# saforem2/l2hmc

Hardware: AMD Instinct MI355X
Metric: leapfrog-steps/sec (whole node), 8x8 U(1) batch 2048, 10 LF (higher is better)
Workload: dtype f32; 1 GPU; U(1) 8x8 lattice, beta=2.0, batch 2048 per GPU, 10 LF steps, GenericNet H=512 (BASELINE.json configs[2]); global_batch=2048, num_steps=10, parallelism=chains sharded over 1 GPU(s) (weak scaling), weights replicated

## Files before the change

include/l2hmc_hip.h:

```cpp
#ifndef L2HMC_HIP_H
#define L2HMC_HIP_H

#include <stddef.h>
#include <stdint.h>

#ifdef __cplusplus
extern "C" {
#endif

#define L2HMC_OK 0
#define L2HMC_ERR_ARG 1
#define L2HMC_ERR_HIP 2
#define L2HMC_ERR_WORKSPACE 3

#define L2HMC_ABI_VERSION 1

typedef void* l2hmc_stream_t;

int l2hmc_abi_version(void);
const char* l2hmc_last_error(void);

int l2hmc_u1_action_force(const float* x, int64_t rows, int32_t T, int32_t X, float beta,
                          float* action, float* force, float* avg_plaq, float* top_charge,
                          l2hmc_stream_t stream);
// ... 38 lines not shown

int l2hmc_stq_dense(const l2hmc_dense_net* net, const float* a, const float* b, const float* bmask,
                    float t_cos, float t_sin, int64_t rows, float* S, float* T, float* Q,
                    void* ws, size_t ws_bytes, l2hmc_stream_t stream);

size_t l2hmc_stq_conv3d_ws_bytes(int64_t rows, int32_t H, int32_t T, int32_t X, int32_t F);
int l2hmc_stq_conv3d(const l2hmc_conv3d_front* front, const l2hmc_dense_net* net, int32_t T, int32_t X,
                     const float* a, const float* b, const float* bmask, float t_cos, float t_sin,
                     int64_t rows, float* S, float* Tr, float* Q, void* ws, size_t ws_bytes,
                     l2hmc_stream_t stream);

int l2hmc_lf_update_v(const float* v, const float* grad, const float* S, const float* T,
                      const float* Q, float eps, int32_t dir, int64_t rows, int32_t D,
                      float* v_out, float* logdet, l2hmc_stream_t stream);
int l2hmc_lf_update_x(const float* x, const float* v, const float* keep, const float* S,
                      const float* T, const float* Q, float eps, int32_t dir, int64_t rows,
                      int32_t D, float* x_out, float* logdet, l2hmc_stream_t stream);

int l2hmc_accept_prob(const float* h_old, const float* h_new, const float* sumlogdet, int64_t n,
                      float* p, l2hmc_stream_t stream);

int l2hmc_mix_accept(const float* x, const float* xf, const float* vf, const float* pf,
                     const float* xb, const float* vb, const float* pb, const float* coin,
                     const float* u, int32_t strict, int64_t B, int32_t D, float* x_prop,
                     float* v_prop, float* p, float* x_out, l2hmc_stream_t stream);

#define L2HMC_PLAN_LAYERED 1
#define L2HMC_PLAN_CONV3D 2
#define L2HMC_PLAN_SELECTED_ONLY 4
#define L2HMC_PLAN_RECOMPUTE 8
#define L2HMC_PLAN_TILES16_ONLY 16
#define L2HMC_PLAN_ALL_COLUMNS 32
#define L2HMC_PLAN_FULL_L1 64
typedef struct l2hmc_gauge_plan {
  int32_t T, X;
  int32_t num_steps;
  int32_t hmc;
  float eps;
  int32_t flags;
  const float* masks;
  l2hmc_dense_net xnet;
  l2hmc_dense_net vnet;
  l2hmc_conv3d_front xfront;
  l2hmc_conv3d_front vfront;
  const void* heads;
} l2hmc_gauge_plan;

size_t l2hmc_gauge_pack_heads_bytes(const l2hmc_gauge_plan* plan);
int l2hmc_gauge_pack_heads(const l2hmc_gauge_plan* plan, void* heads, l2hmc_stream_t stream);

size_t l2hmc_gauge_ws_bytes(const l2hmc_gauge_plan* plan, int64_t rows);

int l2hmc_gauge_plan_fused(const l2hmc_gauge_plan* plan);

int l2hmc_gauge_step_plan(int64_t rows_all, int32_t cus, int64_t* rows_out, int32_t* rows_per_wg_out);

int l2hmc_gauge_leapfrog(const l2hmc_gauge_plan* plan, float beta, int32_t step, float* x, float* v,
                         const int32_t* dir, int64_t rows, float* logdet, void* ws, size_t ws_bytes,
                         l2hmc_stream_t stream);

int l2hmc_gauge_trajectory(const l2hmc_gauge_plan* plan, float beta, const float* x0, const float* v0,
                           const int32_t* dir, int64_t rows, float* x_out, float* v_out,
                           float* sumlogdet, float* p_accept, void* ws, size_t ws_bytes,
                           l2hmc_stream_t stream);

size_t l2hmc_gauge_transition_ws_bytes(const l2hmc_gauge_plan* plan, int64_t B, int32_t both_directions);
// ... 178 lines not shown
```

l2hmc_amd/_lib.py:

```python
import ctypes as C
import os
import re

import torch

_HERE = os.path.dirname(os.path.abspath(__file__))
LIB_PATH = os.environ.get("L2HMC_LIB_PATH") or os.path.join(_HERE, "libl2hmc_hip.so")
HEADER_PATH = os.path.join(os.path.dirname(_HERE), "include", "l2hmc_hip.h")

c_float_p = C.c_void_p
MAX_MIX, MAX_SMALL_DIM, MAX_SMALL_NODES = 8, 8, 64
PLAN_LAYERED, PLAN_CONV3D, PLAN_SELECTED_ONLY, PLAN_RECOMPUTE, PLAN_TILES16_ONLY, PLAN_ALL_COLUMNS = 1, 2, 4, 8, 16, 32
PLAN_FULL_L1 = 64
GRAD_BUCKET_REST = 6
BUCKET_FN = C.CFUNCTYPE(None, C.c_void_p, C.c_int32)


class DenseNet(C.Structure):
    _fields_ = [("D", C.c_int32), ("H", C.c_int32), ("Ka", C.c_int32), ("Kb", C.c_int32),
                ("w1_t", c_float_p), ("wt", c_float_p), ("b1", c_float_p), ("wh_t", c_float_p),
                ("bh", c_float_p), ("whd_t", c_float_p), ("bhd", c_float_p),
                ("coeff_s", c_float_p), ("coeff_q", c_float_p),
                ("q_tanh", C.c_int32), ("reserved", C.c_int32), ("packed", c_float_p)]


class DenseGrads(C.Structure):
    _fields_ = [(n, c_float_p) for n in ("w1_t", "wt", "b1", "wh_t", "bh", "whd_t", "bhd", "coeff_s", "coeff_q")]


class Conv3DGrads(C.Structure):
    _fields_ = [(n, c_float_p) for n in ("w1_a", "b1_a", "w2_a", "b2_a", "w1_b", "b1_b", "w2_b", "b2_b")]


class Conv3DFront(C.Structure):
    _fields_ = [("F", C.c_int32), ("reserved", C.c_int32),
                ("w1_a", c_float_p), ("b1_a", c_float_p), ("w2_a", c_float_p), ("b2_a", c_float_p),
                ("w1_b", c_float_p), ("b1_b", c_float_p), ("w2_b", c_float_p), ("b2_b", c_float_p)]


class GaugePlan(C.Structure):
    _fields_ = [("T", C.c_int32), ("X", C.c_int32), ("num_steps", C.c_int32), ("hmc", C.c_int32),
                ("eps", C.c_float), ("flags", C.c_int32), ("masks", c_float_p),
                ("xnet", DenseNet), ("vnet", DenseNet), ("xfront", Conv3DFront), ("vfront", Conv3DFront),
                ("heads", C.c_void_p)]


# ... 211 lines not shown
```

l2hmc_amd/csrc/fused_args.h:

```cpp
#pragma once
#include "stq_dense.h"

namespace l2hmc {

struct FusedArgs {
  int T, X, num_steps, step_begin, step_end;
  float eps, beta;
  const float* masks;
  l2hmc_dense_net xnet, vnet;
  l2hmc_conv3d_front xfront, vfront;
  const float* x0; const float* v0;
  const int* dir;
  int64_t x_mod;
  int64_t dir_split;
  int64_t rows;
  float* x_out; float* v_out;
  float* logdet;
  int logdet_accumulate;
  float* p_accept;
  unsigned long long* stamps;
  int stagger;
  FusedTape tx, tv;
  float* step_x_next;
  float* step_xprop; float* step_vprop; float* step_xout;
  int64_t step_B;
  int64_t step_Bl, step_chain0;
  int step_sums_acc;
  unsigned long long step_seed, step_draw;
  int step_both;
  float* step_px; float* step_act; float* step_plq; float* step_chg; float* step_dq;
  float* step_sums;
  float* step_part;
  int step_split;
  float* step_hand;
  int* step_ticket;
  const int* heads_meta;
  const float* heads_img;
  const float* l1_img;
};

size_t fused4_pack_floats(const l2hmc_dense_net* n);
int launch_fused4_pack(const l2hmc_dense_net* n, float* image4, hipStream_t stream);
int fused4_rows_per_wg(int64_t rows, int cus);
int launch_fused4(const FusedArgs& a, int rows_per_wg, hipStream_t stream);

int fused32_supported(const l2hmc_dense_net* n);
int launch_fused32(const FusedArgs& a, hipStream_t stream);

}
```

l2hmc_amd/csrc/fused_traj.hip:

```cpp
#include "fused_step.h"
#include "lf_update.h"
#include <atomic>
#include <stdlib.h>

namespace l2hmc {

template <int D, int H, int KA = D, bool CONV = false>
struct FusedCfg {
  static constexpr int IMGW = CONV ? 2 * kFWaves : kFWaves;
  static constexpr int WAVES = 2 * kFWaves;
  static constexpr int RW = WAVES / IMGW;
  static constexpr int THREADS = 64 * WAVES;
  static constexpr int TPC = CONV ? THREADS / kFM : 16;
  static constexpr int SX = D + 8;
  static constexpr int SA = KA + 8;
  static constexpr int SH = H + 8;
  static constexpr int NT1 = H / (16 * WAVES);
  static constexpr int NTH = D / (16 * WAVES);
  static constexpr int NTI1 = H / (16 * IMGW);
  static constexpr int NTIH = D / (16 * IMGW);
  static_assert(NT1 >= 1 && NT1 <= 8 && NTH >= 1, "every wave needs at least one tile per layer");
  static_assert(RW == 1 || NTH == 1, "a shared heads section is walked with one tile per head and wave");
  static constexpr int KC1 = 2 * KA / 16;
  static constexpr int KC2 = H / 16;
  static constexpr size_t P1 = (size_t)2 * KA * H;
  static constexpr size_t P2 = (size_t)H * H;
  static constexpr size_t PH = (size_t)3 * D * H;
  static constexpr int NC = 4 * H + 5 * D;
  static constexpr int CF = 8, CL = 8;
  static constexpr int CW = 18 * CF + CF + 8 * CF * CF + 2 * CF;
  static constexpr int CXIN = (CL + 2) * (CL + 2) * 2;
  static constexpr int CP1 = (CL / 2 + 1) * (CL / 2 + 1) * CF;
  static constexpr int CONV_FLOATS = CONV ? 2 * kFM * SA + 4 * CW + kFM * (CXIN + CP1) : 0;
  static constexpr int ACT_FLOATS = CONV ? 0 : kFM * SX + D + 4 + D + 2 * kFM;
  static constexpr int LDS_FLOATS = 3 * kFM * SX + 2 * kFM * SH + 2 * NC + kFM * (D / 2 + 4)  +
                                    2 * D  + WAVES * kFM  + (RW > 1 ? IMGW * 64 : 0)  + kFM  +
                                    8 * kFM  + CONV_FLOATS + ACT_FLOATS;
};

__global__ void pack_fused_kernel(l2hmc_dense_net n, float* __restrict__ out, int waves) {
  const int kFWaves = waves;
  const int D = n.D, H = n.H, K1 = n.Ka + n.Kb;
  const size_t P1 = (size_t)K1 * H, P2 = (size_t)H * H, PH = (size_t)3 * D * H;
  const int NT1 = H / (16 * kFWaves), NTH = D / (16 * kFWaves);
  for (size_t i = (size_t)blockIdx.x * blockDim.x + threadIdx.x; i < P1 + P2 + PH;
       i += (size_t)gridDim.x * blockDim.x) {
    const int j = (int)(i & 3), lane = (int)((i >> 2) & 63);
    size_t rest;
    float val;
    if (i < P1 + P2) {
      const bool first = i < P1;
      const int K = first ? K1 : H;
      rest = (first ? i : i - P1) >> 8;
      const int t = (int)(rest % NT1);
      rest /= NT1;
      const int KC = K / 16;
      const int kc = (int)(rest % KC), w = (int)(rest / KC);
      const int col = (w * NT1 + t) * 16 + (lane & 15);
      const int k = kc * 16 + (lane >> 4) * 4 + j;
      val = first ? n.w1_t[(size_t)col * K1 + k] : n.wh_t[(size_t)col * H + k];
    } else {
      rest = (i - P1 - P2) >> 8;
      const int t = (int)(rest % NTH);
      rest /= NTH;
      const int hd = (int)(rest % 3);
      rest /= 3;
      const int KC = H / 16;
// ... 86 lines not shown
    __builtin_amdgcn_sched_barrier(0);                                                        \
    t_;                                                                                       \
  })
#define FT_ADD(slot, t0) ft[slot] += FT_NOW() - (t0)
#else
#define FT_NOW() 0ull
#define FT_ADD(slot, t0) do {} while (0)
#endif


#ifdef L2HMC_STAMPS
int g_fused_stagger = 0;
extern "C" void l2hmc_debug_set_stagger(int cycles) { g_fused_stagger = cycles; }
#endif

template <int D, int H, int KA, bool CONV, bool TAPE = false>
__global__ __launch_bounds__((FusedCfg<D, H, KA, CONV>::THREADS)) void gauge_traj_fused_kernel(FusedArgs p) {
  using Cfg = FusedCfg<D, H, KA, CONV>;
  constexpr int kFWaves = Cfg::WAVES, kFThreads = Cfg::THREADS, kTPC = Cfg::TPC;
  constexpr int SX = Cfg::SX, SH = Cfg::SH, SA = Cfg::SA, NT1 = Cfg::NT1, NTH = Cfg::NTH;
  constexpr int RW = Cfg::RW, IMGW = Cfg::IMGW, NTI1 = Cfg::NTI1, NTIH = Cfg::NTIH;
  constexpr int TSH = RW > 1 ? NTIH : 1;
  constexpr int sites = D / 2;
  constexpr int SP = sites + 4;
  extern __shared__ __attribute__((aligned(16))) float lds[];
  float* xs = lds;
  float* vs = xs + kFM * SX;
  float* gs = vs + kFM * SX;
  float* h1 = gs + kFM * SX;
  float* h2 = h1 + kFM * SH;
  float* cx = h2 + kFM * SH;
  float* cv = cx + Cfg::NC;
  float* sp = cv + Cfg::NC;
  float* skm = sp + kFM * SP;
  float* ldw = skm + 2 * D;
  float* ldx = ldw + IMGW * kFM;
  int* sdir = reinterpret_cast<int*>(ldw + kFWaves * kFM + (RW > 1 ? IMGW * 64 : 0));
  float* stp = reinterpret_cast<float*>(sdir + kFM);
  float* fa = stp + 8 * kFM;
  float* fb = fa + kFM * SA;
  float* cwl = fb + kFM * SA;
  float* cxin = cwl + 4 * Cfg::CW;
  float* cp1 = cxin + kFM * Cfg::CXIN;
  float* stg = stp + 8 * kFM + Cfg::CONV_FLOATS;
  int* scol = reinterpret_cast<int*>(stg + kFM * SX);
  int* sel = scol + D;
  int* scp = sel + 4;
  float* spz = reinterpret_cast<float*>(scp + D);

  [[maybe_unused]] unsigned long long ft[10] = {0, 0, 0, 0, 0, 0, 0, 0, 0, 0};
  [[maybe_unused]] const unsigned long long ft_start = FT_NOW();
#ifdef L2HMC_STAMPS
  unsigned long long rt0;
  asm volatile("s_memrealtime %0\n\ts_waitcnt lgkmcnt(0)" : "=s"(rt0)::"memory");
#endif
  const int tid = threadIdx.x;
  const int lane = tid & 63, wave = tid >> 6;
  const int q = lane >> 4, r = lane & 15;
  const int64_t row0 = (int64_t)blockIdx.x * kFM;
  const int nrow = (int)min((int64_t)kFM, p.rows - row0);
  const float eps = p.eps;

#ifdef L2HMC_STAMPS
  if (p.stagger > 0) {
    const long long delay = (long long)((blockIdx.x >> 3) & 31) * p.stagger;
    const long long t0 = (long long)__builtin_amdgcn_s_memtime();
    while ((long long)__builtin_amdgcn_s_memtime() - t0 < delay) __builtin_amdgcn_s_sleep(16);
  }
#endif
  const bool SPLIT = !CONV && !TAPE && p.step_B > 0 && p.step_both && p.step_split;
  const StepWg wg = step_workgroup<kFM>(p, stp, SPLIT);
  const bool STEPM = wg.stepm;
  const int sdw = wg.sdw;
  float* spx = wg.spx;
  stage_chains<kFM, kFThreads, D, SX>(p, wg, xs, vs, sdir);
  load_consts<kFThreads, D, H>(p.xnet, cx, tid);
  load_consts<kFThreads, D, H>(p.vnet, cv, tid);
  if constexpr (CONV) {
    constexpr int F = Cfg::CF, F2 = 2 * Cfg::CF;
    auto load_filters = [&](const float* w1, const float* b1, const float* w2, const float* b2, float* dst) {
      for (int i = tid; i < 18 * F; i += kFThreads) dst[i] = w1[i];
// ... 101 lines not shown
          for (int wi = 0; wi < 3; ++wi)
#pragma unroll
            for (int wj = 0; wj < 3; ++wj)
              w[wi][wj] = *reinterpret_cast<const f32x4*>(pbase + (wi * L2P + wj) * F + ch4);
#pragma unroll
          for (int di = 0; di < 2; ++di)
#pragma unroll
            for (int dj = 0; dj < 2; ++dj)
#pragma unroll
              for (int cc = 0; cc < 4; ++cc) {
                const f32x2 kw = *reinterpret_cast<const f32x2*>(w2 + ((di * 2 + dj) * F + ch4 + cc) * F2 + 2 * gp);
#pragma unroll
                for (int a = 0; a < 2; ++a)
#pragma unroll
                  for (int bb = 0; bb < 2; ++bb) {
                    const float xv = w[a + di][bb + dj][cc];
                    acc[a][bb] += f32x2{xv, xv} * kw;
                  }
              }
        }
        const float m0 = fmaxf(fmaxf(acc[0][0][0], acc[0][1][0]), fmaxf(acc[1][0][0], acc[1][1][0]));
        const float m1 = fmaxf(fmaxf(acc[0][0][1], acc[0][1][1]), fmaxf(acc[1][0][1], acc[1][1][1]));
        *reinterpret_cast<f32x2*>(dst + c * SA + (I2 * L4 + J2) * F2 + 2 * gp) = f32x2{fmaxf(m0, 0.f), fmaxf(m1, 0.f)};
      }
    }
    __syncthreads();
  };

  f32x4 keep_v[NT1], keep_x[NT1];
  bool keep_v_valid = false;
  constexpr bool ACTOK = !CONV && !TAPE && Cfg::NTH == 1 && RW == 2 && kFWaves == 8;
  int arow = 0;

  auto net_update = [&](const l2hmc_dense_net& net, const float* cn, const float* in1, int mode, int sub,
                        bool prep_next_mask, int l1, bool is_vnet, const float tcr, const float tsr,
                        int callidx) {
    const float* pk = net.packed;
    const bool zig = (callidx & 1) != 0;
    [[maybe_unused]] const FusedTape& tp = is_vnet ? p.tv : p.tx;
    [[maybe_unused]] const size_t tcr0 = (size_t)callidx * (size_t)p.rows + (size_t)row0;
    if constexpr (TAPE) {
      {
        const float* stsrc = mode == 1 ? vs : xs;
        for (int i = tid; i < kFM * (D / 4); i += kFThreads) {
          const int rr = i / (D / 4), c4 = (i - rr * (D / 4)) * 4;
          if (rr < nrow) {
            float* dst = tp.in + (tcr0 + rr) * (2 * D);
            tape_store(dst + c4, *reinterpret_cast<const f32x4*>(in1 + rr * SX + c4));
            tape_store(dst + D + c4, *reinterpret_cast<const f32x4*>(gs + rr * SX + c4));
            tape_store(tp.st + (tcr0 + rr) * D + c4, *reinterpret_cast<const f32x4*>(stsrc + rr * SX + c4));
          }
        }
      }
    }
    [[maybe_unused]] auto tape_rows = [&](float* dst, const float* src) {
      for (int i = tid; i < kFM * (H / 4); i += kFThreads) {
        const int rr = i / (H / 4), c4 = (i - rr * (H / 4)) * 4;
        if (rr < nrow)
          tape_store(dst + (tcr0 + rr) * H + c4, *reinterpret_cast<const f32x4*>(src + rr * SH + c4));
      }
    };
    const int wv = __builtin_amdgcn_readfirstlane(wave);
    const int wimg = wv / RW, wsub = wv - wimg * RW;
    const float* wp1 = pk + (size_t)wimg * Cfg::KC1 * NTI1 * 256;
    const float* wp2 = pk + Cfg::P1 + (size_t)wimg * Cfg::KC2 * NTI1 * 256;
    const float* wph = pk + Cfg::P1 + Cfg::P2 + (size_t)wimg * Cfg::KC2 * 3 * NTIH * 256;
    const int to1 = wsub * NT1, toh = wsub * NTH;
    int asense = 0;
    bool actv = false;
    const float* wpa = nullptr;
    if (ACTOK && SPLIT && mode == 2 && p.heads_img) {
      asense = sdw ^ sub;
      actv = __builtin_amdgcn_readfirstlane(sel[asense]) != 0;
      wpa = p.heads_img + ((size_t)(arow * 2 + asense) * 4 + (wv & 3)) * Cfg::KC2 * 3 * 256;
    }
    const bool l1c = ACTOK && SPLIT && p.l1_img && p.heads_img && __builtin_amdgcn_readfirstlane(sel[0] & sel[1]) != 0;
    [[maybe_unused]] float ld_k[4] = {0.f, 0.f, 0.f, 0.f}, ld_s[4] = {0.f, 0.f, 0.f, 0.f};
#ifndef L2HMC_DP1
#define L2HMC_DP1 3
#define L2HMC_DP2 3
#define L2HMC_DPH 4
#endif
    constexpr int DP1 = L2HMC_DP1, DP2 = L2HMC_DP2, DPH = L2HMC_DPH;
    BRing<NT1, DP2> R2;
    BRing<3 * NTH, DPH> R3;
    {
      constexpr int KH = Cfg::KC1 / 2;
      f32x4 acc[NT1];
      [[maybe_unused]] unsigned long long t0 = FT_NOW();
      const float* src1 = in1;
      const float* src2 = gs;
      int s1 = SX;
      if constexpr (CONV) {
        const float* cwn = cwl + (is_vnet ? 2 : 0) * Cfg::CW;
        [[maybe_unused]] const unsigned long long tc0 = FT_NOW();
        if (l1 == 0 || l1 == 1 || l1 == 3) conv_features(in1, cwn, fa);
        if (l1 != 2) conv_features(gs, cwn + Cfg::CW, fb);
        FT_ADD(8, tc0);
        src1 = fa;
        src2 = fb;
        s1 = SA;
        if constexpr (TAPE) {
          for (int i = tid; i < kFM * (2 * KA / 4); i += kFThreads) {
            const int rr = i / (2 * KA / 4), c4 = (i - rr * (2 * KA / 4)) * 4;
            if (rr < nrow)
              tape_store(tp.feat + (tcr0 + rr) * (2 * KA) + c4,
                         *reinterpret_cast<const f32x4*>((c4 < KA ? fa + rr * SA + c4 : fb + rr * SA + (c4 - KA))));
          }
        }
      }
      if (l1 == 2) {
#pragma unroll
        for (int t = 0; t < NT1; ++t) acc[t] = keep_v[t];
      } else {
        BRing<NT1, DP1> RA, RB;
        const bool cmp = l1c && mode == 2;
        const float* wpb = wp1 + (size_t)KH * NTI1 * 256;
        if (cmp) wpb = p.l1_img + ((size_t)(arow * 2 + asense) * IMGW + wimg) * (KH / 2) * NTI1 * 256;
        ring_prime<NT1, DP1, NTI1>(RB, wpb, false, 0, to1);
        if (l1 == 4) {
#pragma unroll
          for (int t = 0; t < NT1; ++t) acc[t] = keep_x[t];
// ... 8 lines not shown
#pragma unroll
            for (int t = 0; t < NT1; ++t) keep_x[t] = acc[t];
          }
        }
        bool x_done = false;
        if constexpr (ACTOK) {
          if (cmp) {
            x_done = true;
            const float* a2 = (sub == 0 ? stg : gs) + r * SX + q * 4;
            const bool bad = spz[sub * kFM + r] != 0.f;
            stream_layer<NT1, KH / 2, DP1, NTI1>(
                RB, wpb,
                [&](int kc) {
                  f32x4 a = *reinterpret_cast<const f32x4*>(a2 + kc * 16);
                  if (kc == 0) {
#pragma unroll
                    for (int e = 0; e < 4; ++e) a[e] = bad ? __builtin_nanf("") : a[e];
                  }
                  return a;
                },
                acc, false, to1);
          }
        }
        if (!x_done) {
          const float* a2 = src2 + r * s1 + q * 4;
          stream_layer<NT1, KH, DP1, NTI1>(
              RB, wpb, [&](int kc) { return *reinterpret_cast<const f32x4*>(a2 + kc * 16); }, acc, false, to1);
        }
        if (l1 == 1) {
#pragma unroll
          for (int t = 0; t < NT1; ++t) keep_v[t] = acc[t];
        }
      }
      ring_prime<NT1, DP2, NTI1>(R2, wp2, zig, Cfg::KC2, to1);
      FT_ADD(0, t0);
      t0 = FT_NOW();
      [[maybe_unused]] unsigned gmask = 0;
#pragma unroll
      for (int t = 0; t < NT1; ++t) {
        const int c0 = (wave * NT1 + t) * 16 + q * 4;
        const f32x4 b = *reinterpret_cast<const f32x4*>(cn + c0);
        const f32x4 w0 = *reinterpret_cast<const f32x4*>(cn + H + c0);
        const f32x4 w1 = *reinterpret_cast<const f32x4*>(cn + 2 * H + c0);
        f32x4 hv;
#pragma unroll
        for (int e = 0; e < 4; ++e) {
          hv[e] = fmaxf(acc[t][e] + b[e] + (tcr * w0[e] + tsr * w1[e]), 0.f);
          if constexpr (TAPE) gmask |= (hv[e] > 0.f ? 1u : 0u) << (t * 4 + e);
        }
        *reinterpret_cast<f32x4*>(h1 + r * SH + c0) = hv;
      }
      if constexpr (TAPE) {
        const size_t word = ((size_t)(callidx * 2 + 0) * gridDim.x + blockIdx.x) * (64 * IMGW) + wimg * 64 + lane;
        if constexpr (RW == 1) tp.gate[word] = gmask;
        else reinterpret_cast<unsigned short*>(tp.gate)[word * 2 + wsub] = (unsigned short)gmask;
      }
      FT_ADD(3, t0);
    }
    {
      [[maybe_unused]] const unsigned long long tb = FT_NOW();
      __syncthreads();
      FT_ADD(6, tb);
    }
    if constexpr (TAPE) tape_rows(tp.h1, h1);
    {
      f32x4 acc[NT1];
#pragma unroll
      for (int t = 0; t < NT1; ++t) acc[t] = f32x4{0.f, 0.f, 0.f, 0.f};
      const float* a = h1 + r * SH + q * 4;
      [[maybe_unused]] unsigned long long t0 = FT_NOW();
      stream_layer<NT1, Cfg::KC2, DP2, NTI1>(
          R2, wp2, [&](int kc) { return *reinterpret_cast<const f32x4*>(a + kc * 16); }, acc, zig, to1);
      if (ACTOK && actv) {
        if (wv < 4) ring_prime<3 * NTH, DPH, 3, 1>(R3, wpa, zig, Cfg::KC2, 0);
      } else {
        ring_prime<3 * NTH, DPH, 3 * NTIH, TSH>(R3, wph, zig, Cfg::KC2, toh);
      }
      FT_ADD(1, t0);
      t0 = FT_NOW();
      [[maybe_unused]] unsigned gmask = 0;
#pragma unroll
      for (int t = 0; t < NT1; ++t) {
        const int c0 = (wave * NT1 + t) * 16 + q * 4;
        const f32x4 b = *reinterpret_cast<const f32x4*>(cn + 3 * H + c0);
        f32x4 hv;
#pragma unroll
        for (int e = 0; e < 4; ++e) {
          hv[e] = fmaxf(acc[t][e] + b[e], 0.f);
          if constexpr (TAPE) gmask |= (hv[e] > 0.f ? 1u : 0u) << (t * 4 + e);
        }
        *reinterpret_cast<f32x4*>(h2 + r * SH + c0) = hv;
      }
      if constexpr (TAPE) {
        const size_t word = ((size_t)(callidx * 2 + 1) * gridDim.x + blockIdx.x) * (64 * IMGW) + wimg * 64 + lane;
        if constexpr (RW == 1) tp.gate[word] = gmask;
        else reinterpret_cast<unsigned short*>(tp.gate)[word * 2 + wsub] = (unsigned short)gmask;
      }
      FT_ADD(4, t0);
    }
    {
      [[maybe_unused]] const unsigned long long tb = FT_NOW();
      __syncthreads();
      FT_ADD(6, tb);
    }
    if constexpr (TAPE) tape_rows(tp.h2, h2);
    {
      f32x4 acc[3 * NTH];
#pragma unroll
      for (int t = 0; t < 3 * NTH; ++t) acc[t] = f32x4{0.f, 0.f, 0.f, 0.f};
      const float* a = h2 + r * SH + q * 4;
      [[maybe_unused]] unsigned long long t0 = FT_NOW();
      if (ACTOK && actv) {
        if (wv < 4)
          stream_layer<3 * NTH, Cfg::KC2, DPH, 3, 1>(
              R3, wpa, [&](int kc) { return *reinterpret_cast<const f32x4*>(a + kc * 16); }, acc, zig, 0);
      } else {
        stream_layer<3 * NTH, Cfg::KC2, DPH, 3 * NTIH, TSH>(
            R3, wph, [&](int kc) { return *reinterpret_cast<const f32x4*>(a + kc * 16); }, acc, zig, toh);
      }
      FT_ADD(2, t0);
      t0 = FT_NOW();
      float ld = 0.f;
      const float* bhd = cn + 4 * H;
      const float* es = bhd + 3 * D;
      const float* eq = es + D;
      const int d = dirl;
      if (ACTOK && actv) {
        const int* al = scol + asense * (D / 2);
        const int* il = scol + (asense ^ 1) * (D / 2);
        if (wv < 4) {
#pragma unroll
          for (int e = 0; e < 4; ++e) {
            const int c = al[wv * 16 + q * 4 + e];
            const int idx = r * SX + c;
            float S, Tt, Q, s, omk;
            heads_stq(acc[0][e], acc[1][e], acc[2][e], bhd[c], bhd[D + c], bhd[2 * D + c], es[c], eq[c], net.q_tanh, S,
                      Tt, Q);
            const float xn = lf_drift<ExpFast>(xs[idx], vs[idx], keep_of(skm[c], skm[D + c], d, sub), S, Tt, Q, eps, d, s,
                                               omk);
            xs[idx] = xn;
            stg[idx] = omk * s;
            if (prep_next_mask) gs[l1c ? r * SX + scp[c] : idx] = omk * xn;
          }
        } else {
#pragma unroll
          for (int e = 0; e < 4; ++e) {
            const int c = il[(wv - 4) * 16 + q * 4 + e];
            const int idx = r * SX + c;
            stg[idx] = 0.f;
            if (prep_next_mask) {
              const float kx = (1.f - keep_of(skm[c], skm[D + c], d, sub)) * xs[idx];
              if (!l1c) gs[idx] = kx;
              else if (kx != kx) spz[kFM + r] = kx;
// ... 82 lines not shown
      }
      }
      FT_ADD(5, t0);
    }
    {
      [[maybe_unused]] const unsigned long long tb = FT_NOW();
      __syncthreads();
      FT_ADD(6, tb);
    }
    if (ACTOK && actv) {
      if (wsub == 1) {
        float ld = 0.f;
#pragma unroll
        for (int h = 0; h < 2; ++h)
#pragma unroll
          for (int e = 0; e < 4; ++e) ld += stg[r * SX + (2 * wimg + h) * 16 + q * 4 + e];
        ld += __shfl_xor(ld, 16, 64);
        ld += __shfl_xor(ld, 32, 64);
        if (q == 0) ldw[wimg * kFM + r] += ld;
      }
    } else if constexpr (RW > 1) {
      if (wsub == 1) {
        float ld = ldx[wimg * 64 + lane];
#pragma unroll
        for (int e = 0; e < 4; ++e) ld += ld_k[e] * ld_s[e];
        ld += __shfl_xor(ld, 16, 64);
        ld += __shfl_xor(ld, 32, 64);
        if (q == 0) ldw[wimg * kFM + r] += ld;
      }
    }
  };

  const float two_pi = 6.28318530717958647692f;
  for (int step = p.step_begin; step < p.step_end; ++step) {
    const int sf = step, sb = p.num_steps - 1 - step;
    const float af = two_pi * (float)sf / (float)p.num_steps, ab = two_pi * (float)sb / (float)p.num_steps;
    const float tcf = cosf(af), tsf = sinf(af), tcb = cosf(ab), tsb = sinf(ab);
    const float tcr = dirl ? tcb : tcf, tsr = dirl ? tsb : tsf;
    for (int i = tid; i < D; i += kFThreads) {
      skm[i] = p.masks[(size_t)sf * D + i];
      skm[D + i] = p.masks[(size_t)sb * D + i];
    }
    if (ACTOK && SPLIT && p.heads_meta) {
      arow = sdw ? sb : sf;
      for (int i = tid; i < D; i += kFThreads) scol[i] = p.heads_meta[2 * p.num_steps + arow * D + i];
      if (tid < 2) sel[tid] = p.heads_meta[arow * 2 + tid];
      if (p.l1_img)
        for (int i = tid; i < D; i += kFThreads) scp[i] = p.heads_meta[2 * p.num_steps + (p.num_steps + arow) * D + i];
    }
    __syncthreads();
#pragma nounroll
    for (int call = 0; call < 4; ++call) {
      const bool is_v = call == 0 || call == 3;
      if (call == 3) {
        [[maybe_unused]] const unsigned long long tf = FT_NOW();
        float unused[1];
        force_pass<kFM, kTPC, 1, D, SX, SP>(cl, xs, sp, gs, unused);
        FT_ADD(7, tf);
      }
      const int l1 = call == 0 ? (keep_v_valid ? 2 : 0) : call == 1 ? 3 : call == 2 ? 4 : 1;
      net_update(is_v ? p.vnet : p.xnet, is_v ? cv : cx, is_v ? xs : vs, is_v ? 1 : 2, call == 2 ? 1 : 0,
                 call < 2, l1, is_v, tcr, tsr, 2 * step + (call == 0 || call == 1 ? 0 : 1));
    }
    keep_v_valid = true;
  }

  float act1[1], kin1[1];
  force_pass<kFM, kTPC, 1, D, SX, SP>(cl, xs, sp, gs, act1);
  kinetic_pass<kFM, kTPC, 1, D, SX>(cl, vs, kin1);
  if (STEPM) {
    step_accept_probs<kFM, 1, IMGW>(cl, ldw, act0, act1, kin0, kin1, spx);
    __syncthreads();
    const float* xfr = xs;
    const float* xbr = xs + (kFM / 2) * SX;
    const float* vfr = vs;
    const float* vbr = vs + (kFM / 2) * SX;
    const float* pfr = spx;
    const float* pbr = spx + kFM / 2;
    if (SPLIT) {
      constexpr int HW = 2 * kFM * D + kFM;
      float* mine = p.step_hand + (size_t)blockIdx.x * HW;
      for (int i = tid; i < kFM * (D / 4); i += kFThreads) {
        const int rr = i / (D / 4), c4 = (i - rr * (D / 4)) * 4;
        *reinterpret_cast<f32x4*>(mine + rr * D + c4) = *reinterpret_cast<const f32x4*>(xs + rr * SX + c4);
        if (p.step_vprop)
          *reinterpret_cast<f32x4*>(mine + (kFM + rr) * D + c4) = *reinterpret_cast<const f32x4*>(vs + rr * SX + c4);
      }
      if (tid < kFM) mine[2 * kFM * D + tid] = spx[tid];
      asm volatile("s_waitcnt vmcnt(0)" ::: "memory");
      int* is_last = sdir;
      __syncthreads();
      if (tid == 0) {
        __builtin_amdgcn_fence(__ATOMIC_RELEASE, "agent");
        asm volatile("s_waitcnt vmcnt(0)" ::: "memory");
        const int got = __hip_atomic_fetch_add(p.step_ticket + (blockIdx.x >> 1), 1, __ATOMIC_RELAXED,
                                               __HIP_MEMORY_SCOPE_AGENT);
        if (got == 1) {
// ... 76 lines not shown
  if (p->hmc || !p->xnet.packed || !p->vnet.packed || 2 * p->T * p->X != 128 || (p->X & (p->X - 1)) != 0) return 0;
  if (p->flags & L2HMC_PLAN_CONV3D)
    return fused_conv_net(&p->xnet) && fused_conv_net(&p->vnet) && p->T == 8 && p->X == 8 && p->xfront.F == 8 &&
           p->vfront.F == 8;
  return fused_generic_net(&p->xnet) && fused_generic_net(&p->vnet);
}

int launch_fused_trajectory(const l2hmc_gauge_plan* p, float beta, int step_begin, int step_end,
                            const float* x0, const float* v0, const int* dir, int64_t rows, float* x_out,
                            float* v_out, float* logdet, int logdet_accumulate, float* p_accept,
                            hipStream_t stream, int64_t x_mod, int64_t dir_split, const FusedTape* tape_x,
                            const FusedTape* tape_v) {
  const bool conv = (p->flags & L2HMC_PLAN_CONV3D) != 0;
  using CfgG = FusedCfg<128, 512, 128, false>;
  using CfgC = FusedCfg<128, 256, 64, true>;
  static DeviceOnce attr_once;
  const bool tape = tape_x && tape_v;
  const size_t lds = sizeof(float) * (conv ? CfgC::LDS_FLOATS : CfgG::LDS_FLOATS);
  if (attr_once.pending()) {
    if (hipFuncSetAttribute(reinterpret_cast<const void*>(&gauge_traj_fused_kernel<128, 512, 128, false>),
                            hipFuncAttributeMaxDynamicSharedMemorySize,
                            (int)(sizeof(float) * CfgG::LDS_FLOATS)) != hipSuccess ||
        hipFuncSetAttribute(reinterpret_cast<const void*>(&gauge_traj_fused_kernel<128, 256, 64, true>),
                            hipFuncAttributeMaxDynamicSharedMemorySize,
                            (int)(sizeof(float) * CfgC::LDS_FLOATS)) != hipSuccess) {
      set_error("fused trajectory: cannot reserve %zu B of LDS", lds);
      return L2HMC_ERR_HIP;
    }
    attr_once.done();
  }
  FusedArgs a{};
  a.T = p->T; a.X = p->X; a.num_steps = p->num_steps; a.step_begin = step_begin; a.step_end = step_end;
  a.eps = p->eps; a.beta = beta; a.masks = p->masks; a.xnet = p->xnet; a.vnet = p->vnet;
  a.xfront = p->xfront; a.vfront = p->vfront;
  a.x0 = x0; a.v0 = v0; a.dir = dir; a.rows = rows; a.x_out = x_out; a.v_out = v_out;
  a.x_mod = x_mod; a.dir_split = dir_split;
  a.logdet = logdet; a.logdet_accumulate = logdet_accumulate; a.p_accept = p_accept;
  if (tape) {
    L2HMC_REQUIRE(step_begin == 0, "fused trajectory: taping needs the whole trajectory");
    L2HMC_REQUIRE(!conv || (tape_x->feat && tape_v->feat), "fused trajectory: ConvNet3D taping needs the feature tape");
    L2HMC_REQUIRE(tape_x->in && tape_x->h1 && tape_x->h2 && tape_x->stq && tape_x->st && tape_v->in && tape_v->h1 &&
                      tape_v->h2 && tape_v->stq && tape_v->st && tape_x->gate && tape_v->gate,
                  "fused trajectory: NULL tape pointer");
    a.tx = *tape_x;
    a.tv = *tape_v;
    static DeviceOnce tape_once;
    if (tape_once.pending()) {
      if (hipFuncSetAttribute(reinterpret_cast<const void*>(&gauge_traj_fused_kernel<128, 512, 128, false, true>),
                              hipFuncAttributeMaxDynamicSharedMemorySize,
                              (int)(sizeof(float) * CfgG::LDS_FLOATS)) != hipSuccess ||
          hipFuncSetAttribute(reinterpret_cast<const void*>(&gauge_traj_fused_kernel<128, 256, 64, true, true>),
                              hipFuncAttributeMaxDynamicSharedMemorySize,
                              (int)(sizeof(float) * CfgC::LDS_FLOATS)) != hipSuccess) {
        set_error("fused trajectory: cannot reserve %zu B of LDS", lds);
        return L2HMC_ERR_HIP;
      }
      tape_once.done();
    }
  }
#ifdef L2HMC_STAMPS
  a.stamps = g_stamp_cls == 5 ? g_stamp_buf : nullptr;
  a.stagger = g_fused_stagger;
#endif
  if (!conv && !tape && subtile_enabled(p)) {
    if (const int rpw = fused4_rows_per_wg(rows, device_cu_count())) return launch_fused4(a, rpw, stream);
    if (rows > (int64_t)kFM * device_cu_count()) return launch_fused32(a, stream);
// ... 60 lines not shown
}

int launch_fused_step(const l2hmc_gauge_plan* p, float beta, const float* x_in, float* x_next, int64_t B,
                      uint64_t seed, uint64_t draw, int both, float* px, float* actions, float* plaqs, float* charges,
                      float* dq, float* step_sums, float* part, void* hand, hipStream_t stream, float* x_prop,
                      float* v_prop, float* x_out) {
  const bool conv = (p->flags & L2HMC_PLAN_CONV3D) != 0;
  using CfgG = FusedCfg<128, 512, 128, false>;
  using CfgC = FusedCfg<128, 256, 64, true>;
  static DeviceOnce step_once;
  const size_t lds = sizeof(float) * (conv ? CfgC::LDS_FLOATS : CfgG::LDS_FLOATS);
  if (step_once.pending()) {
    if (hipFuncSetAttribute(reinterpret_cast<const void*>(&gauge_traj_fused_kernel<128, 512, 128, false>),
                            hipFuncAttributeMaxDynamicSharedMemorySize,
                            (int)(sizeof(float) * CfgG::LDS_FLOATS)) != hipSuccess ||
        hipFuncSetAttribute(reinterpret_cast<const void*>(&gauge_traj_fused_kernel<128, 256, 64, true>),
                            hipFuncAttributeMaxDynamicSharedMemorySize,
                            (int)(sizeof(float) * CfgC::LDS_FLOATS)) != hipSuccess) {
      set_error("fused step: cannot reserve %zu B of LDS", lds);
      return L2HMC_ERR_HIP;
    }
    step_once.done();
  }
  L2HMC_REQUIRE(x_in && (x_next || x_out) && B > 0 && (!step_sums || part) && hand, "fused step: bad arguments");
  const int ndir = both ? 2 : 1;
  StepPart parts[3];
  const int nparts = plan_step_parts(B * ndir, !conv && subtile_enabled(p), device_cu_count(), parts);
  auto part_of = [&](int64_t c0, int64_t nb, int rpw, int accumulate) {
    const int cpw = both ? rpw / 2 : rpw;
    const int64_t D = 2 * (int64_t)p->T * p->X;
    FusedArgs a{};
    a.T = p->T; a.X = p->X; a.num_steps = p->num_steps; a.step_begin = 0; a.step_end = p->num_steps;
    a.eps = p->eps; a.beta = beta; a.masks = p->masks; a.xnet = p->xnet; a.vnet = p->vnet;
    a.xfront = p->xfront; a.vfront = p->vfront;
    a.x0 = x_in + c0 * D; a.rows = ceil_div(nb, cpw) * rpw;
    a.step_x_next = x_next ? x_next + c0 * D : nullptr;
    a.step_xprop = x_prop ? x_prop + c0 * D : nullptr;
    a.step_vprop = v_prop ? v_prop + c0 * D : nullptr;
    a.step_xout = x_out ? x_out + c0 * D : nullptr;
    a.step_B = B; a.step_Bl = nb; a.step_chain0 = c0; a.step_sums_acc = accumulate;
    a.step_seed = seed; a.step_draw = draw; a.step_both = both;
    a.step_px = px ? px + c0 : nullptr; a.step_act = actions ? actions + c0 : nullptr;
    a.step_plq = plaqs ? plaqs + c0 : nullptr; a.step_chg = charges ? charges + c0 : nullptr;
    a.step_dq = dq ? dq + c0 : nullptr;
    a.step_sums = step_sums; a.step_part = part;
#ifdef L2HMC_STAMPS
    a.stamps = g_stamp_cls == 5 ? g_stamp_buf : nullptr;
    a.stagger = g_fused_stagger;
#endif
    return a;
  };
  const bool split = !conv && both;
  const int* hmeta = nullptr;
  const float* himg = nullptr;
  const float* l1img = nullptr;
  if (split && p->heads && !(p->flags & L2HMC_PLAN_ALL_COLUMNS)) {
    const int Dp = 2 * p->T * p->X;
    hmeta = reinterpret_cast<const int*>(p->heads);
    himg = reinterpret_cast<const float*>(reinterpret_cast<const char*>(p->heads) + heads_meta_bytes(p->num_steps, Dp));
    if (!(p->flags & L2HMC_PLAN_FULL_L1))
      l1img = reinterpret_cast<const float*>(reinterpret_cast<const char*>(himg) +
                                             heads_sections_bytes(p->num_steps, Dp, p->xnet.H));
  }
  auto launch16 = [&](FusedArgs a) {
    if (split) {
      const int64_t pairs = ceil_div(a.step_Bl, (int64_t)kFM);
// ... 82 lines not shown
```

l2hmc_amd/gauge_dynamics.py:

```python
import ctypes as C

import numpy as np
import numpy.random as npr
import torch

from . import _lib, ops
from . import autograd as _autograd
from .network import ConvNet3D, GenericNet


class GaugeDynamics:

    def __init__(self, lattice, potential_fn, **kwargs):
        self.name = 'GaugeDynamics'
        self.lattice = lattice
        self.potential = potential_fn
        self.batch_size = self.lattice.samples.shape[0]
        self.x_dim = self.lattice.num_links
        self.hmc, self.network_arch, self.num_steps = False, 'generic', 5
        self.eps_trainable, self.data_format = True, 'channels_last'
        self.both_directions = True
        self.fused = True
        self.check_numerics = False
        self.recompute = False
        self.tiles16_only = False
        self.all_columns = False
        self.full_l1 = False
        for key, val in kwargs.items():
            if key != 'eps':
                setattr(self, key, val)
        self._device = kwargs.get('device') or torch.device("cuda", torch.cuda.current_device())
        if getattr(potential_fn, "u1_lattice", None) is None:
            raise NotImplementedError(
                "the fused trajectory integrates the 2D U(1) action; pass lattice.get_energy_function()")
        self.eps = torch.tensor(float(kwargs.get('eps', 0.4)), dtype=torch.float32)
        self._construct_time()
        self._construct_masks_while()
        if self.hmc:
            self.position_fn = lambda inp: [torch.zeros_like(inp[0]) for _ in range(3)]
            self.momentum_fn = lambda inp: [torch.zeros_like(inp[0]) for _ in range(3)]
        elif self.network_arch == 'generic':
            self._build_generic_nets()
        elif self.network_arch == 'conv3D':
            self._build_conv_nets_3D()
        elif self.network_arch == 'conv2D':
            raise NotImplementedError(
                "network_arch='conv2D' is out of scope (SURVEY.md section 2: not named by any benchmark "
                "config, and its 4-D outputs break the reference's own reduce_sum(axis=1))")
        else:
            raise AttributeError("`self._network_arch` must be one of `'conv3D', 'conv2D', 'generic'.`")
        self._ws = _lib.Workspace()
        self._seed = int(kwargs.get('seed', 42))
        self._draws = 0

    def _build_generic_nets(self):
        kwargs = {'x_dim': self.x_dim, 'links_shape': self.lattice.links.shape,
                  'num_hidden': int(4 * self.x_dim), 'name_scope': 'position', 'factor': 2.}
        self.position_fn = GenericNet(model_name='XNet', device=self._device, **kwargs)
        kwargs['factor'] = 1.
        kwargs['name_scope'] = 'momentum'
# ... 29 lines not shown
            mask = np.zeros((self.x_dim,))
            mask[idx] = 1
            mask_per_step.append(mask)
        self.set_masks(np.stack(mask_per_step))

    def set_masks(self, masks):
        masks = np.asarray(masks, dtype=np.float32)
        if masks.shape != (self.num_steps, self.x_dim):
            raise ValueError(f"masks: expected {(self.num_steps, self.x_dim)}, got {masks.shape}")
        self.mask = _lib.as_dev(masks, self._device)

    @property
    def variables(self):
        v = [self.eps]
        if not self.hmc:
            v += self.position_fn.variables + self.momentum_fn.variables
        return v

    @property
    def trainable_variables(self):
        v = [self.eps] if self.eps_trainable else []
        if not self.hmc:
            v += self.position_fn.trainable_variables + self.momentum_fn.trainable_variables
        return v

    def _plan(self):
        p = _lib.GaugePlan(T=self.lattice.time_size, X=self.lattice.space_size, num_steps=self.num_steps,
                           hmc=int(bool(self.hmc)), eps=float(self.eps.detach()),
                           flags=(0 if self.fused else _lib.PLAN_LAYERED)
                           | (0 if self.both_directions else _lib.PLAN_SELECTED_ONLY)
                           | (_lib.PLAN_RECOMPUTE if self.recompute else 0)
                           | (_lib.PLAN_TILES16_ONLY if self.tiles16_only else 0)
                           | (_lib.PLAN_ALL_COLUMNS if self.all_columns else 0)
                           | (_lib.PLAN_FULL_L1 if self.full_l1 else 0),
                           masks=_lib.dev_ptr(self.mask, name="mask"))
        if not self.hmc:
            p.xnet = self.position_fn.pack()
            p.vnet = self.momentum_fn.pack()
            if self.network_arch == 'conv3D':
                p.flags |= _lib.PLAN_CONV3D
                p.xfront = self.position_fn.pack_front()
                p.vfront = self.momentum_fn.pack_front()
            elif self.fused:
                p.heads = self._heads_image(p)
        return p

    def _heads_image(self, plan):
        L = _lib.lib()
        nbytes = L.l2hmc_gauge_pack_heads_bytes(C.byref(plan))
        if not nbytes:
            return None
        key = (plan.xnet.whd_t, getattr(self.position_fn, "_pack_serial", 0))
        h = getattr(self, "_heads", None)
        if h is None or h[0] is not self.mask or h[1] != key or h[2].numel() * 4 < nbytes:
            buf = torch.empty(nbytes // 4, dtype=torch.float32, device=self._device)
            _lib.call("l2hmc_gauge_pack_heads", C.byref(plan), buf, device=self._device)
            self._heads = h = (self.mask, key, buf)
        return h[2].data_ptr()

    def _x(self, a):
        a = _lib.as_dev(a, self._device)
        return a.reshape(a.shape[0], -1)

    def _normal(self, shape):
        out = ops.fill_normal(shape, self._seed, self._draws, self._device)
        self._draws += 1
        return out
# ... 134 lines not shown
```

Measured before the change: 15.75 million chain-leapfrog-steps/s.

## Overlap next-step mask fetch and first-layer epilogue across leapfrog step boundary

Inside the fused trajectory kernel, the step-boundary work is pipelined. The mask and heads-metadata rows for step+1 are prefetched during the previous step's heads-layer streaming into a double-buffered LDS set. The next step's first vnet layer-1 epilogue is folded into the last call of the current step, so the following step enters directly at layer 2. This removes a serial global load plus __syncthreads and an epilogue pass at each step edge. The cost is extra LDS for the second mask buffer and more complex control flow, and a new plan flag restores the serial path.

```diff
diff --git a/include/l2hmc_hip.h b/include/l2hmc_hip.h
--- a/include/l2hmc_hip.h
+++ b/include/l2hmc_hip.h
@@ -94,6 +94,7 @@
 #define L2HMC_PLAN_TILES16_ONLY 16
 #define L2HMC_PLAN_ALL_COLUMNS 32
 #define L2HMC_PLAN_FULL_L1 64
+#define L2HMC_PLAN_SERIAL_STEP_EDGE 128
 typedef struct l2hmc_gauge_plan {
   int32_t T, X;
   int32_t num_steps;
diff --git a/l2hmc_amd/_lib.py b/l2hmc_amd/_lib.py
--- a/l2hmc_amd/_lib.py
+++ b/l2hmc_amd/_lib.py
@@ -12,6 +12,7 @@
 MAX_MIX, MAX_SMALL_DIM, MAX_SMALL_NODES = 8, 8, 64
 PLAN_LAYERED, PLAN_CONV3D, PLAN_SELECTED_ONLY, PLAN_RECOMPUTE, PLAN_TILES16_ONLY, PLAN_ALL_COLUMNS = 1, 2, 4, 8, 16, 32
 PLAN_FULL_L1 = 64
+PLAN_SERIAL_STEP_EDGE = 128
 GRAD_BUCKET_REST = 6
 BUCKET_FN = C.CFUNCTYPE(None, C.c_void_p, C.c_int32)
 
diff --git a/l2hmc_amd/csrc/fused_args.h b/l2hmc_amd/csrc/fused_args.h
--- a/l2hmc_amd/csrc/fused_args.h
+++ b/l2hmc_amd/csrc/fused_args.h
@@ -37,6 +37,7 @@
   const int* heads_meta;
   const float* heads_img;
   const float* l1_img;
+  int serial_step_edge;
 };
 
 size_t fused4_pack_floats(const l2hmc_dense_net* n);
diff --git a/l2hmc_amd/csrc/fused_traj.hip b/l2hmc_amd/csrc/fused_traj.hip
--- a/l2hmc_amd/csrc/fused_traj.hip
+++ b/l2hmc_amd/csrc/fused_traj.hip
@@ -32,7 +32,8 @@
   static constexpr int CXIN = (CL + 2) * (CL + 2) * 2;
   static constexpr int CP1 = (CL / 2 + 1) * (CL / 2 + 1) * CF;
   static constexpr int CONV_FLOATS = CONV ? 2 * kFM * SA + 4 * CW + kFM * (CXIN + CP1) : 0;
-  static constexpr int ACT_FLOATS = CONV ? 0 : kFM * SX + D + 4 + D + 2 * kFM;
+  static constexpr int MSK2_FLOATS = 2 * D + D + 4 + D;
+  static constexpr int ACT_FLOATS = CONV ? 0 : kFM * SX + D + 4 + D + 2 * kFM + MSK2_FLOATS;
   static constexpr int LDS_FLOATS = 3 * kFM * SX + 2 * kFM * SH + 2 * NC + kFM * (D / 2 + 4)  +
                                     2 * D  + WAVES * kFM  + (RW > 1 ? IMGW * 64 : 0)  + kFM  +
                                     8 * kFM  + CONV_FLOATS + ACT_FLOATS;
@@ -185,8 +186,8 @@
   float* cx = h2 + kFM * SH;
   float* cv = cx + Cfg::NC;
   float* sp = cv + Cfg::NC;
-  float* skm = sp + kFM * SP;
-  float* ldw = skm + 2 * D;
+  float* const skm0 = sp + kFM * SP;
+  float* ldw = skm0 + 2 * D;
   float* ldx = ldw + IMGW * kFM;
   int* sdir = reinterpret_cast<int*>(ldw + kFWaves * kFM + (RW > 1 ? IMGW * 64 : 0));
   float* stp = reinterpret_cast<float*>(sdir + kFM);
@@ -196,10 +197,15 @@
   float* cxin = cwl + 4 * Cfg::CW;
   float* cp1 = cxin + kFM * Cfg::CXIN;
   float* stg = stp + 8 * kFM + Cfg::CONV_FLOATS;
-  int* scol = reinterpret_cast<int*>(stg + kFM * SX);
+  int* const scol0 = reinterpret_cast<int*>(stg + kFM * SX);
+  float* spz = reinterpret_cast<float*>(scol0 + D + 4 + D);
+  float* const skm1 = spz + 2 * kFM;
+  int* const scol1 = reinterpret_cast<int*>(skm1 + 2 * D);
+  int mset = 0;
+  float* skm = skm0;
+  int* scol = scol0;
   int* sel = scol + D;
   int* scp = sel + 4;
-  float* spz = reinterpret_cast<float*>(scp + D);
 
   [[maybe_unused]] unsigned long long ft[10] = {0, 0, 0, 0, 0, 0, 0, 0, 0, 0};
   [[maybe_unused]] const unsigned long long ft_start = FT_NOW();
@@ -367,9 +373,37 @@
   constexpr bool ACTOK = !CONV && !TAPE && Cfg::NTH == 1 && RW == 2 && kFWaves == 8;
   int arow = 0;
 
+  static_assert(kFThreads >= 4 * D, "one mask word per thread");
+  struct MaskRows { float km; int meta, ok; };
+  auto fetch_masks = [&](int step) {
+    const int sf = step, sb = p.num_steps - 1 - step;
+    MaskRows m{0.f, 0, 0};
+    if (tid < D) m.km = p.masks[(size_t)sf * D + tid];
+    else if (tid < 2 * D) m.km = p.masks[(size_t)sb * D + (tid - D)];
+    if (ACTOK && SPLIT && p.heads_meta) {
+      const int ar = sdw ? sb : sf;
+      if (tid >= 2 * D && tid < 3 * D) m.meta = p.heads_meta[2 * p.num_steps + ar * D + (tid - 2 * D)];
+      else if (tid >= 3 * D && tid < 4 * D && p.l1_img)
+        m.meta = p.heads_meta[2 * p.num_steps + (p.num_steps + ar) * D + (tid - 3 * D)];
+      if (tid < 2) m.ok = p.heads_meta[ar * 2 + tid];
+    }
+    return m;
+  };
+  auto store_masks = [&](const MaskRows& m, float* km, int* col) {
+    if (tid < 2 * D) km[tid] = m.km;
+    if (ACTOK && SPLIT && p.heads_meta) {
+      if (tid >= 2 * D && tid < 3 * D) col[tid - 2 * D] = m.meta;
+      else if (tid >= 3 * D && tid < 4 * D && p.l1_img) col[D + 4 + (tid - 3 * D)] = m.meta;
+      if (tid < 2) col[D + tid] = m.ok;
+    }
+  };
+  constexpr bool EDGEOK = !CONV && !TAPE;
+  const bool edge = EDGEOK && !p.serial_step_edge;
+  float tcn = 0.f, tsn = 0.f;
+
   auto net_update = [&](const l2hmc_dense_net& net, const float* cn, const float* in1, int mode, int sub,
                         bool prep_next_mask, int l1, bool is_vnet, const float tcr, const float tsr,
-                        int callidx) {
+                        int callidx, bool enter_l2, int fetch_step, bool fold_next) {
     const float* pk = net.packed;
     const bool zig = (callidx & 1) != 0;
     [[maybe_unused]] const FusedTape& tp = is_vnet ? p.tv : p.tx;
@@ -419,10 +453,29 @@
     constexpr int DP1 = L2HMC_DP1, DP2 = L2HMC_DP2, DPH = L2HMC_DPH;
     BRing<NT1, DP2> R2;
     BRing<3 * NTH, DPH> R3;
+    auto l1_epilogue = [&](const f32x4 (&pre)[NT1], const float tc, const float ts) {
+      unsigned gmask = 0;
+#pragma unroll
+      for (int t = 0; t < NT1; ++t) {
+        const int c0 = (wave * NT1 + t) * 16 + q * 4;
+        const f32x4 b = *reinterpret_cast<const f32x4*>(cn + c0);
+        const f32x4 w0 = *reinterpret_cast<const f32x4*>(cn + H + c0);
+        const f32x4 w1 = *reinterpret_cast<const f32x4*>(cn + 2 * H + c0);
+        f32x4 hv;
+#pragma unroll
+        for (int e = 0; e < 4; ++e) {
+          hv[e] = fmaxf(pre[t][e] + b[e] + (tc * w0[e] + ts * w1[e]), 0.f);
+          if constexpr (TAPE) gmask |= (hv[e] > 0.f ? 1u : 0u) << (t * 4 + e);
+        }
+        *reinterpret_cast<f32x4*>(h1 + r * SH + c0) = hv;
+      }
+      return gmask;
+    };
     {
-      constexpr int KH = Cfg::KC1 / 2;
       f32x4 acc[NT1];
       [[maybe_unused]] unsigned long long t0 = FT_NOW();
+      if (!enter_l2) {
+      constexpr int KH = Cfg::KC1 / 2;
       const float* src1 = in1;
       const float* src2 = gs;
       int s1 = SX;
@@ -497,35 +550,24 @@
           for (int t = 0; t < NT1; ++t) keep_v[t] = acc[t];
         }
       }
+      }
       ring_prime<NT1, DP2, NTI1>(R2, wp2, zig, Cfg::KC2, to1);
       FT_ADD(0, t0);
+      if (!enter_l2) {
       t0 = FT_NOW();
-      [[maybe_unused]] unsigned gmask = 0;
-#pragma unroll
-      for (int t = 0; t < NT1; ++t) {
-        const int c0 = (wave * NT1 + t) * 16 + q * 4;
-        const f32x4 b = *reinterpret_cast<const f32x4*>(cn + c0);
-        const f32x4 w0 = *reinterpret_cast<const f32x4*>(cn + H + c0);
-        const f32x4 w1 = *reinterpret_cast<const f32x4*>(cn + 2 * H + c0);
-        f32x4 hv;
-#pragma unroll
-        for (int e = 0; e < 4; ++e) {
-          hv[e] = fmaxf(acc[t][e] + b[e] + (tcr * w0[e] + tsr * w1[e]), 0.f);
-          if constexpr (TAPE) gmask |= (hv[e] > 0.f ? 1u : 0u) << (t * 4 + e);
-        }
-        *reinterpret_cast<f32x4*>(h1 + r * SH + c0) = hv;
-      }
+      [[maybe_unused]] const unsigned gmask = l1_epilogue(acc, tcr, tsr);
       if constexpr (TAPE) {
         const size_t word = ((size_t)(callidx * 2 + 0) * gridDim.x + blockIdx.x) * (64 * IMGW) + wimg * 64 + lane;
         if constexpr (RW == 1) tp.gate[word] = gmask;
         else reinterpret_cast<unsigned short*>(tp.gate)[word * 2 + wsub] = (unsigned short)gmask;
       }
       FT_ADD(3, t0);
-    }
-    {
-      [[maybe_unused]] const unsigned long long tb = FT_NOW();
-      __syncthreads();
-      FT_ADD(6, tb);
+      {
+        [[maybe_unused]] const unsigned long long tb = FT_NOW();
+        __syncthreads();
+        FT_ADD(6, tb);
+      }
+      }
     }
     if constexpr (TAPE) tape_rows(tp.h1, h1);
     {
@@ -575,6 +617,10 @@
       for (int t = 0; t < 3 * NTH; ++t) acc[t] = f32x4{0.f, 0.f, 0.f, 0.f};
       const float* a = h2 + r * SH + q * 4;
       [[maybe_unused]] unsigned long long t0 = FT_NOW();
+      MaskRows nxt{0.f, 0, 0};
+      if constexpr (EDGEOK) {
+        if (fetch_step >= 0) nxt = fetch_masks(fetch_step);
+      }
       if (ACTOK && actv) {
         if (wv < 4)
           stream_layer<3 * NTH, Cfg::KC2, DPH, 3, 1>(
@@ -584,6 +630,14 @@
             R3, wph, [&](int kc) { return *reinterpret_cast<const f32x4*>(a + kc * 16); }, acc, zig, toh);
       }
       FT_ADD(2, t0);
+      if constexpr (EDGEOK) {
+        if (fetch_step >= 0) store_masks(nxt, mset ? skm0 : skm1, mset ? scol0 : scol1);
+        if (fold_next) {
+          t0 = FT_NOW();
+          l1_epilogue(keep_v, tcn, tsn);
+          FT_ADD(3, t0);
+        }
+      }
       t0 = FT_NOW();
       float ld = 0.f;
       const float* bhd = cn + 4 * H;
@@ -732,23 +786,35 @@
   };
 
   const float two_pi = 6.28318530717958647692f;
+  bool folded = false;
+  float tcr = 0.f, tsr = 0.f;
   for (int step = p.step_begin; step < p.step_end; ++step) {
-    const int sf = step, sb = p.num_steps - 1 - step;
-    const float af = two_pi * (float)sf / (float)p.num_steps, ab = two_pi * (float)sb / (float)p.num_steps;
-    const float tcf = cosf(af), tsf = sinf(af), tcb = cosf(ab), tsb = sinf(ab);
-    const float tcr = dirl ? tcb : tcf, tsr = dirl ? tsb : tsf;
-    for (int i = tid; i < D; i += kFThreads) {
-      skm[i] = p.masks[(size_t)sf * D + i];
-      skm[D + i] = p.masks[(size_t)sb * D + i];
-    }
-    if (ACTOK && SPLIT && p.heads_meta) {
-      arow = sdw ? sb : sf;
-      for (int i = tid; i < D; i += kFThreads) scol[i] = p.heads_meta[2 * p.num_steps + arow * D + i];
-      if (tid < 2) sel[tid] = p.heads_meta[arow * 2 + tid];
-      if (p.l1_img)
-        for (int i = tid; i < D; i += kFThreads) scp[i] = p.heads_meta[2 * p.num_steps + (p.num_steps + arow) * D + i];
-    }
-    __syncthreads();
+    tcr = tcn;
+    tsr = tsn;
+#pragma nounroll
+    for (int k = step == p.step_begin ? 0 : 1; k < 2; ++k) {
+      const int sf = step + k, sb = p.num_steps - 1 - sf;
+      const float af = two_pi * (float)sf / (float)p.num_steps, ab = two_pi * (float)sb / (float)p.num_steps;
+      const float tcf = cosf(af), tsf = sinf(af), tcb = cosf(ab), tsb = sinf(ab);
+      tcn = dirl ? tcb : tcf;
+      tsn = dirl ? tsb : tsf;
+      if (k == 0) {
+        tcr = tcn;
+        tsr = tsn;
+      }
+    }
+    if (ACTOK && SPLIT && p.heads_meta) arow = sdw ? p.num_steps - 1 - step : step;
+    if (folded) {
+      mset ^= 1;
+      skm = mset ? skm1 : skm0;
+      scol = mset ? scol1 : scol0;
+      sel = scol + D;
+      scp = sel + 4;
+    } else {
+      store_masks(fetch_masks(step), skm, scol);
+      __syncthreads();
+    }
+    const bool has_next = edge && step + 1 < p.step_end;
 #pragma nounroll
     for (int call = 0; call < 4; ++call) {
       const bool is_v = call == 0 || call == 3;
@@ -760,9 +826,11 @@
       }
       const int l1 = call == 0 ? (keep_v_valid ? 2 : 0) : call == 1 ? 3 : call == 2 ? 4 : 1;
       net_update(is_v ? p.vnet : p.xnet, is_v ? cv : cx, is_v ? xs : vs, is_v ? 1 : 2, call == 2 ? 1 : 0,
-                 call < 2, l1, is_v, tcr, tsr, 2 * step + (call == 0 || call == 1 ? 0 : 1));
+                 call < 2, l1, is_v, tcr, tsr, 2 * step + (call == 0 || call == 1 ? 0 : 1), call == 0 && folded,
+                 call == 2 && has_next ? step + 1 : -1, call == 3 && has_next);
     }
     keep_v_valid = true;
+    folded = has_next;
   }
 
   float act1[1], kin1[1];
@@ -905,6 +973,7 @@
   FusedArgs a{};
   a.T = p->T; a.X = p->X; a.num_steps = p->num_steps; a.step_begin = step_begin; a.step_end = step_end;
   a.eps = p->eps; a.beta = beta; a.masks = p->masks; a.xnet = p->xnet; a.vnet = p->vnet;
+  a.serial_step_edge = (p->flags & L2HMC_PLAN_SERIAL_STEP_EDGE) != 0;
   a.xfront = p->xfront; a.vfront = p->vfront;
   a.x0 = x0; a.v0 = v0; a.dir = dir; a.rows = rows; a.x_out = x_out; a.v_out = v_out;
   a.x_mod = x_mod; a.dir_split = dir_split;
@@ -1031,6 +1100,7 @@
     FusedArgs a{};
     a.T = p->T; a.X = p->X; a.num_steps = p->num_steps; a.step_begin = 0; a.step_end = p->num_steps;
     a.eps = p->eps; a.beta = beta; a.masks = p->masks; a.xnet = p->xnet; a.vnet = p->vnet;
+    a.serial_step_edge = (p->flags & L2HMC_PLAN_SERIAL_STEP_EDGE) != 0;
     a.xfront = p->xfront; a.vfront = p->vfront;
     a.x0 = x_in + c0 * D; a.rows = ceil_div(nb, cpw) * rpw;
     a.step_x_next = x_next ? x_next + c0 * D : nullptr;
diff --git a/l2hmc_amd/gauge_dynamics.py b/l2hmc_amd/gauge_dynamics.py
--- a/l2hmc_amd/gauge_dynamics.py
+++ b/l2hmc_amd/gauge_dynamics.py
@@ -26,6 +26,7 @@
         self.tiles16_only = False
         self.all_columns = False
         self.full_l1 = False
+        self.serial_step_edge = False
         for key, val in kwargs.items():
             if key != 'eps':
                 setattr(self, key, val)
@@ -121,7 +122,8 @@
                            | (_lib.PLAN_RECOMPUTE if self.recompute else 0)
                            | (_lib.PLAN_TILES16_ONLY if self.tiles16_only else 0)
                            | (_lib.PLAN_ALL_COLUMNS if self.all_columns else 0)
-                           | (_lib.PLAN_FULL_L1 if self.full_l1 else 0),
+                           | (_lib.PLAN_FULL_L1 if self.full_l1 else 0)
+                           | (_lib.PLAN_SERIAL_STEP_EDGE if self.serial_step_edge else 0),
                            masks=_lib.dev_ptr(self.mask, name="mask"))
         if not self.hmc:
             p.xnet = self.position_fn.pack()
```

Result: no change. 15.87 million chain-leapfrog-steps/s (median of 6 runs) (+0.7%).
